# kocvara/Loraine.jl

Hardware: AMD Instinct MI355X
Metric: ms/IP-iteration (Schur assembly + solve), dense SDP n=2000 m=4000 (lower is better)
Workload: dtype f64; 1 GPU; C4 synthetic dense SDP, matrix side 2000, 4000 constraints, kit=0 (assembly + Cholesky + predictor/corrector solves); msz=2000, nvar=4000, seed=20250614, parallelism=1 GPU

## Files before the change

include/loraine_hip.h:

```cpp
#ifndef LORAINE_HIP_H
#define LORAINE_HIP_H

#include <stdint.h>

#ifdef __cplusplus
extern "C" {
#endif

typedef struct lrn_ctx lrn_ctx;

int lrn_create(lrn_ctx** out, int device);
int lrn_destroy(lrn_ctx* ctx);
const char* lrn_last_error(lrn_ctx* ctx);
int lrn_version(void);
int lrn_device_count(void);

int lrn_upload_model(lrn_ctx* ctx, int nlmi, int nvar, const int64_t* msizes,
                     const int64_t* const* AA_colptr, const int64_t* const* AA_rowval,
                     const double* const* AA_nzval,
                     const int64_t* const* B_colptr, const int64_t* const* B_rowval,
                     const double* const* B_nzval,
                     const int64_t* sigmaA, const int64_t* qA,
                     int nlin, const int64_t* Clin_colptr, const int64_t* Clin_rowval,
                     const double* Clin_nzval);
// ... 30 lines not shown
int lrn_matvec(lrn_ctx* ctx, const double* x, double* Ax);
int lrn_matvec_partial(lrn_ctx* ctx, const double* x, double* Ax_partial);
int lrn_prec_setup(lrn_ctx* ctx, int prec, int erank, int aamat, int* info);
int lrn_prec_apply(lrn_ctx* ctx, const double* x, double* Mx);
int lrn_pcg(lrn_ctx* ctx, const double* h, double tol, int maxit, double* x, int* exit_code,
            int* iters);

int lrn_ip_set_c(lrn_ctx* ctx, int ilmi, const double* C);
int lrn_ip_set_iterate(lrn_ctx* ctx, int ilmi, const double* X, const double* S);
int lrn_ip_get_iterate(lrn_ctx* ctx, int ilmi, double* X, double* S);
int lrn_ip_add_diag(lrn_ctx* ctx, int ilmi, int which, double eps);
int lrn_ip_prepare_w(lrn_ctx* ctx, int ilmi, int* info);
int lrn_ip_aa_x(lrn_ctx* ctx, double* out);
int lrn_ip_residual_d(lrn_ctx* ctx, const double* y);
int lrn_ip_rhs_pred(lrn_ctx* ctx, double* out);
int lrn_ip_rhs_pred2(lrn_ctx* ctx, double* aax_out, double* out);
int lrn_ip_rhs_corr(lrn_ctx* ctx, double sigma_mu, double* out);
int lrn_ip_find_step(lrn_ctx* ctx, int predict, double sigma_mu, double tau, const double* dely,
                     double* alpha, double* beta);
int lrn_ip_update(lrn_ctx* ctx, int predict, const double* alpha, const double* beta, double* trXnSn);
int lrn_ip_stats(lrn_ctx* ctx, double* out5);
int lrn_dbg_eigmin(lrn_ctx* ctx, int n, const double* M, double* lam, int* steps);
int lrn_dbg_lanczos(lrn_ctx* ctx, int n, int k, const double* M, double* lam_top, double* U_top,
                    double* lam_min, double* trace, int* steps);

int lrn_dbg_get_block(lrn_ctx* ctx, int il, const char* name, double* out, int* flag);
int lrn_dbg_tridiag_eig(int m, const double* a, const double* b, int k, const double* upper, double width, double* eig,
                        int64_t* evals);

typedef int (*lrn_host_allreduce_fn)(void* user, double* buf, int64_t count, int op);
typedef int (*lrn_host_allgather_fn)(void* user, const double* send, double* recv, int64_t count_per_rank);
int lrn_comm_unique_id(void* id128);
int lrn_comm_init(lrn_ctx* ctx, const void* id128, int rank, int world);
int lrn_comm_init_host(lrn_ctx* ctx, int rank, int world, lrn_host_allreduce_fn allreduce,
                       lrn_host_allgather_fn allgather, void* user);
int lrn_comm_destroy(lrn_ctx* ctx);
int lrn_comm_allreduce(lrn_ctx* ctx, double* buf, int64_t count, int op);

int lrn_get_timing(lrn_ctx* ctx, const char* key, double* ms);
int64_t lrn_get_count(lrn_ctx* ctx, const char* key);
int lrn_mfma_f64_peak(lrn_ctx* ctx, double* tflops);
int lrn_xcc_probe(lrn_ctx* ctx, int nx, int nz, int hold_us, int32_t* out);
int lrn_hbm_copy_peak(lrn_ctx* ctx, int64_t bytes, double* gbps);

int lrn_dbg_gemm(lrn_ctx* ctx, int transA, int transB, int M, int N, int K, double alpha,
                 const double* A, int lda, const double* B, int ldb, double beta, double* C,
                 int ldc, int flags, int ksplit);
int lrn_dbg_product(lrn_ctx* ctx, int kind, int n, const double* A, const double* Bm, double alpha, double a, int tri,
                    double* out0, double* out1, double* scalar);
int lrn_dbg_gemm_plan(int transA, int transB, int M, int N, int K, int lda, int ldb, double beta, int ldc, int flags,
                      int ksplit, int* out6);
int lrn_dbg_schur_chol_plan(int msz, int nd, int rank, int world, int64_t pcap_hint, const int* opts6, int64_t* out10, int* kb,
                            int* ke, int* weights, double* shares3);
int lrn_dbg_mfma_probe(lrn_ctx* ctx, const double* A16x4, const double* B4x16, double* D16x16);
int lrn_dbg_potrf(lrn_ctx* ctx, int n, double* A, int* info);
int lrn_dbg_potrs(lrn_ctx* ctx, int n, const double* A, const double* b, double* x, int* info);
int lrn_dbg_trsm(lrn_ctx* ctx, int n, int nrhs, int trans, const double* A, double* B, int* info);
int lrn_dbg_svd_jacobi(lrn_ctx* ctx, int n, const double* A, double* U_sigma, double* V,
                       double* sigma, int* sweeps);

#ifdef __cplusplus
}
#endif
#endif
```

loraine.jl_amd/_capi.py:

```python
import ctypes as C
import os
import shutil
import subprocess
import sys

import numpy as np

_HERE = os.path.dirname(os.path.abspath(__file__))
LIB_PATH = os.path.join(_HERE, "libloraine_hip.so")

c_ctx = C.c_void_p
PD = C.POINTER(C.c_double)
PI64 = C.POINTER(C.c_int64)
PI = C.POINTER(C.c_int)
PPD = C.POINTER(C.c_void_p)

SIGNATURES = {
    "lrn_create": (C.c_int, [C.POINTER(c_ctx), C.c_int]),
    "lrn_destroy": (C.c_int, [c_ctx]),
    "lrn_last_error": (C.c_char_p, [c_ctx]),
    "lrn_version": (C.c_int, []),
    "lrn_device_count": (C.c_int, []),
    "lrn_upload_model": (C.c_int, [c_ctx, C.c_int, C.c_int, C.c_void_p, PPD, PPD, PPD, PPD, PPD, PPD,
                                   C.c_void_p, C.c_void_p, C.c_int, C.c_void_p, C.c_void_p, C.c_void_p]),
# ... 10 lines not shown
    "lrn_set_lin": (C.c_int, [c_ctx, C.c_void_p, C.c_void_p]),
    "lrn_schur_assemble": (C.c_int, [c_ctx, C.c_int, C.c_void_p]),
    "lrn_schur_get": (C.c_int, [c_ctx, C.c_void_p]),
    "lrn_schur_add_diag": (C.c_int, [c_ctx, C.c_double]),
    "lrn_schur_factor": (C.c_int, [c_ctx, PI]),
    "lrn_schur_solve": (C.c_int, [c_ctx, C.c_void_p, C.c_void_p]),
    "lrn_schur_shard_doubles": (C.c_int64, [c_ctx]),
    "lrn_schur_export_shard": (C.c_int, [c_ctx, C.c_void_p]),
    "lrn_schur_import_all": (C.c_int, [c_ctx, C.c_void_p]),
    "lrn_schur_is_partial_sum": (C.c_int, [c_ctx]),
    "lrn_schur_plan": (C.c_int, [c_ctx, C.c_int, PI]),
    "lrn_schur_export_full": (C.c_int, [c_ctx, C.c_void_p]),
    "lrn_schur_import_full": (C.c_int, [c_ctx, C.c_void_p]),
    "lrn_make_rhs": (C.c_int, [c_ctx, C.c_void_p, PPD, C.c_void_p]),
    "lrn_matvec": (C.c_int, [c_ctx, C.c_void_p, C.c_void_p]),
    "lrn_matvec_partial": (C.c_int, [c_ctx, C.c_void_p, C.c_void_p]),
    "lrn_prec_setup": (C.c_int, [c_ctx, C.c_int, C.c_int, C.c_int, PI]),
    "lrn_prec_apply": (C.c_int, [c_ctx, C.c_void_p, C.c_void_p]),
    "lrn_pcg": (C.c_int, [c_ctx, C.c_void_p, C.c_double, C.c_int, C.c_void_p, PI, PI]),
    "lrn_comm_unique_id": (C.c_int, [C.c_void_p]),
    "lrn_comm_init": (C.c_int, [c_ctx, C.c_void_p, C.c_int, C.c_int]),
    "lrn_comm_init_host": (C.c_int, [c_ctx, C.c_int, C.c_int, C.c_void_p, C.c_void_p, C.c_void_p]),
    "lrn_comm_destroy": (C.c_int, [c_ctx]),
    "lrn_comm_allreduce": (C.c_int, [c_ctx, C.c_void_p, C.c_int64, C.c_int]),
    "lrn_ip_set_c": (C.c_int, [c_ctx, C.c_int, C.c_void_p]),
    "lrn_ip_set_iterate": (C.c_int, [c_ctx, C.c_int, C.c_void_p, C.c_void_p]),
    "lrn_ip_get_iterate": (C.c_int, [c_ctx, C.c_int, C.c_void_p, C.c_void_p]),
    "lrn_ip_add_diag": (C.c_int, [c_ctx, C.c_int, C.c_int, C.c_double]),
    "lrn_ip_prepare_w": (C.c_int, [c_ctx, C.c_int, PI]),
    "lrn_ip_aa_x": (C.c_int, [c_ctx, C.c_void_p]),
    "lrn_ip_residual_d": (C.c_int, [c_ctx, C.c_void_p]),
    "lrn_ip_rhs_pred": (C.c_int, [c_ctx, C.c_void_p]),
    "lrn_ip_rhs_pred2": (C.c_int, [c_ctx, C.c_void_p, C.c_void_p]),
    "lrn_ip_rhs_corr": (C.c_int, [c_ctx, C.c_double, C.c_void_p]),
    "lrn_ip_find_step": (C.c_int, [c_ctx, C.c_int, C.c_double, C.c_double, C.c_void_p, C.c_void_p, C.c_void_p]),
    "lrn_ip_update": (C.c_int, [c_ctx, C.c_int, C.c_void_p, C.c_void_p, C.c_void_p]),
    "lrn_ip_stats": (C.c_int, [c_ctx, C.c_void_p]),
    "lrn_dbg_get_block": (C.c_int, [c_ctx, C.c_int, C.c_char_p, C.c_void_p, PI]),
    "lrn_dbg_tridiag_eig": (C.c_int, [C.c_int, C.c_void_p, C.c_void_p, C.c_int, C.c_void_p, C.c_double, PD, PI64]),
    "lrn_dbg_eigmin": (C.c_int, [c_ctx, C.c_int, C.c_void_p, PD, PI]),
    "lrn_dbg_lanczos": (C.c_int, [c_ctx, C.c_int, C.c_int, C.c_void_p, C.c_void_p, C.c_void_p, PD, PD, PI]),
    "lrn_get_timing": (C.c_int, [c_ctx, C.c_char_p, PD]),
    "lrn_get_count": (C.c_int64, [c_ctx, C.c_char_p]),
    "lrn_mfma_f64_peak": (C.c_int, [c_ctx, PD]),
    "lrn_hbm_copy_peak": (C.c_int, [c_ctx, C.c_int64, PD]),
    "lrn_xcc_probe": (C.c_int, [c_ctx, C.c_int, C.c_int, C.c_int, C.c_void_p]),
    "lrn_dbg_gemm": (C.c_int, [c_ctx, C.c_int, C.c_int, C.c_int, C.c_int, C.c_int, C.c_double, C.c_void_p,
                               C.c_int, C.c_void_p, C.c_int, C.c_double, C.c_void_p, C.c_int, C.c_int, C.c_int]),
    "lrn_dbg_product": (C.c_int, [c_ctx, C.c_int, C.c_int, C.c_void_p, C.c_void_p, C.c_double, C.c_double, C.c_int,
                                  C.c_void_p, C.c_void_p, PD]),
    "lrn_dbg_gemm_plan": (C.c_int, [C.c_int, C.c_int, C.c_int, C.c_int, C.c_int, C.c_int, C.c_int, C.c_double, C.c_int,
                                    C.c_int, C.c_int, PI]),
    "lrn_dbg_schur_chol_plan": (C.c_int, [C.c_int, C.c_int, C.c_int, C.c_int, C.c_int64, PI, PI64, PI, PI, PI, PD]),
    "lrn_dbg_mfma_probe": (C.c_int, [c_ctx, C.c_void_p, C.c_void_p, C.c_void_p]),
    "lrn_dbg_potrf": (C.c_int, [c_ctx, C.c_int, C.c_void_p, PI]),
    "lrn_dbg_potrs": (C.c_int, [c_ctx, C.c_int, C.c_void_p, C.c_void_p, C.c_void_p, PI]),
    "lrn_dbg_trsm": (C.c_int, [c_ctx, C.c_int, C.c_int, C.c_int, C.c_void_p, C.c_void_p, PI]),
    "lrn_dbg_svd_jacobi": (C.c_int, [c_ctx, C.c_int, C.c_void_p, C.c_void_p, C.c_void_p, C.c_void_p, PI]),
}

GEMM_TRI_LOWER, GEMM_TRI_UPPER, GEMM_OFFDIAG_X2, GEMM_SQUARE, GEMM_KSEG_TRI, GEMM_SMALL_TILE = 1, 2, 4, 8, 16, 32
GEMM_KFROM_N, GEMM_KFROM_M, GEMM_KTO_N, GEMM_KTO_M, GEMM_C_MIRROR, GEMM_DYN_MASKS = 64, 128, 1024, 2048, 4096, 131072

_lib = None


class LoraineHipError(RuntimeError):
    pass


def load_library():
    global _lib
    if _lib is not None:
        return _lib
    if not os.path.exists(LIB_PATH) and shutil.which("hipcc") and os.environ.get("LRN_NO_AUTOBUILD") is None:
        csrc = os.path.join(os.path.dirname(os.path.abspath(__file__)), "csrc")
        import fcntl
        with open(os.path.join(csrc, ".build.lock"), "w") as lock:
            fcntl.flock(lock, fcntl.LOCK_EX)
            if not os.path.exists(LIB_PATH):
                print(f"[loraine.jl_amd] {LIB_PATH} missing: running `make -C {csrc}` (hipcc --offload-arch=gfx950)",
                      file=sys.stderr, flush=True)
                subprocess.run(["make", "-C", csrc, "-j8"], check=False, stdout=subprocess.DEVNULL)
    if not os.path.exists(LIB_PATH):
        raise LoraineHipError(
            f"{LIB_PATH} not found: build it with `python -c 'import __graft_entry__ as g; g.build()'` "
            "(hipcc --offload-arch=gfx950). There is no CPU fallback.")
    try:
        import torch
    except ImportError:
        pass
    lib = C.CDLL(LIB_PATH)
    for name, (res, args) in SIGNATURES.items():
        fn = getattr(lib, name)
        fn.restype = res
        fn.argtypes = args
    _lib = lib
    return lib


def ptr(a):
    if a is None:
        return None
    if isinstance(a, int):
        return C.c_void_p(a)
    if isinstance(a, np.ndarray):
        return C.c_void_p(a.ctypes.data)
    if hasattr(a, "data_ptr"):
        if getattr(a, "is_cuda", False):
            import torch
            torch.cuda.current_stream(a.device).synchronize()
        return C.c_void_p(a.data_ptr())
    raise TypeError(type(a))


# ... 10 lines not shown
```

loraine.jl_amd/csrc/api.hip:

```cpp
#include <cstring>

#include "../../include/loraine_hip.h"
#include "ctx.h"
#include "ops.h"
#include "schur_plan.h"

using namespace lrn;

void lrn_free_model(lrn_ctx* c);
namespace lrn {
void prec_free(lrn_ctx* c);
}

extern "C" {

int lrn_version(void) { return 102; }

int lrn_device_count(void) {
  int n = 0;
  if (hipGetDeviceCount(&n) != hipSuccess) {
    (void)hipGetLastError();
    return 0;
  }
  return n;
}

int lrn_create(lrn_ctx** out, int device) {
  if (!out) return LRN_ERR_ARG;
  *out = nullptr;
  int n = lrn_device_count();
  if (n <= 0 || device < 0 || device >= n) return LRN_ERR_HIP;
  if (hipSetDevice(device) != hipSuccess) return LRN_ERR_HIP;
  lrn_ctx* c = new lrn_ctx();
  c->device = device;
  c->profile = false;
  if (hipStreamCreateWithFlags(&c->stream, hipStreamNonBlocking) != hipSuccess ||
      hipEventCreate(&c->ev0) != hipSuccess || hipEventCreate(&c->ev1) != hipSuccess) {
    delete c;
    return LRN_ERR_HIP;
  }
  *out = c;
  return LRN_OK;
}

int lrn_destroy(lrn_ctx* c) {
  if (!c) return LRN_OK;
  (void)hipSetDevice(c->device);
  (void)hipStreamSynchronize(c->stream);
  prec_free(c);
  comm_free(c);
  lrn_free_model(c);
  release(c->info_dev);
  release(c->scratch);
  release(c->jscratch);
  release(c->redbuf);
  release(c->redout);
  release(c->lzbuf);
  release(c->lzbuf2);
  release(c->lxbuf);
  release(c->ezbuf);
  release(c->commvec);
  release(c->commmat);
  release(c->hopbuf);
  release(c->triw);
  release(c->cgpart);
  if (c->pin) (void)hipHostFree(c->pin);
  for (hipEvent_t e : c->pcg_ev) if (e) (void)hipEventDestroy(e);
  (void)hipEventDestroy(c->ev0);
  (void)hipEventDestroy(c->ev1);
  if (c->evA) (void)hipEventDestroy(c->evA);
  if (c->evB) (void)hipEventDestroy(c->evB);
  (void)hipStreamDestroy(c->stream);
  if (c->stream2) (void)hipStreamDestroy(c->stream2);
  if (c->stream3) (void)hipStreamDestroy(c->stream3);
  delete c;
  return LRN_OK;
}

const char* lrn_last_error(lrn_ctx* c) {
  if (!c) return "null context";
  if (const char* g = lrn::gemm_last_error()) {
    if (c->err.find(g) == std::string::npos) c->err += std::string(c->err.empty() ? "" : " | ") + g;
  }
  return c->err.c_str();
}

int lrn_set_option(lrn_ctx* c, const char* key, double value) {
  if (!c || !key) return LRN_ERR_ARG;
  if (!strcmp(key, "dense_threshold")) c->opt.dense_threshold = value;
  else if (!strcmp(key, "profile")) c->profile = value != 0.0;
  else if (!strcmp(key, "t_batch")) { c->opt.t_batch = (long)value; for (auto& b : c->lmi) b.t_cap = b.p_cap = 0; }
  else if (!strcmp(key, "p_batch")) { c->opt.p_batch = (long)value; for (auto& b : c->lmi) b.t_cap = b.p_cap = 0; }
  else if (!strcmp(key, "prec_eig")) c->opt.prec_eig = (int)value;
  else if (!strcmp(key, "pivot_boost")) c->opt.pivot_boost = value;
  else if (!strcmp(key, "schur_chol")) c->opt.schur_chol = (int)value;
  else if (!strcmp(key, "schur_plan")) c->opt.schur_plan = (int)value;
  else if (!strcmp(key, "gemm3_ksplit")) c->opt.gemm3_ksplit = (int)value;
  else if (!strcmp(key, "gemm_no_skip")) c->opt.gemm_no_skip = (int)value;
  else if (!strcmp(key, "gemm_dyn_masks")) c->opt.gemm_dyn_masks = (int)value;
  else if (!strcmp(key, "gemm1_diag")) c->opt.gemm1_diag = (int)value;
  else if (!strcmp(key, "gemm_lab")) c->opt.gemm_lab = (int)value & 127;
  else if (!strcmp(key, "gemm3_sched")) c->opt.gemm3_sched = (int)value;
  else if (!strcmp(key, "gemm3_tile")) c->opt.gemm3_tile = (int)value;
  else if (!strcmp(key, "gemm3_strip")) c->opt.gemm3_strip = (int)value;
  else if (!strcmp(key, "gemm3_stagger")) c->opt.gemm3_stagger = (int)value;
  else if (!strcmp(key, "jacobi_wgs")) c->opt.jacobi_wgs = (int)value;
  else if (!strcmp(key, "jacobi_block")) c->opt.jacobi_block = (int)value;
  else if (!strcmp(key, "jacobi_inner")) c->opt.jacobi_inner = (int)value;
  else if (!strcmp(key, "pair_lanes")) c->opt.pair_lanes = (int)value;
  else if (!strcmp(key, "matvec_sparse")) c->opt.matvec_sparse = (int)value;
  else if (!strcmp(key, "prec_dense")) c->opt.prec_dense = (int)value;
  else if (!strcmp(key, "wmw_pattern_min")) c->opt.wmw_pattern_min = std::max(2, (int)value);
  else if (!strcmp(key, "profile_symv")) c->opt.profile_symv = (int)value;
  else if (!strcmp(key, "profile_ops")) c->opt.profile_ops = (int)value;
  else if (!strcmp(key, "matvec_h")) { c->opt.matvec_h = (int)value; c->hop_version = -1; }
  else if (!strcmp(key, "comm_fail_ensure")) lrn::comm_inject_ensure_failure(c);
  else if (!strcmp(key, "pcg_lookahead")) c->opt.pcg_lookahead = std::max(0, std::min(8, (int)value));
  else if (!strcmp(key, "lowrank_form")) c->opt.lowrank_form = std::max(-1, std::min(1, (int)value));
  else if (!strcmp(key, "cg_lowrank")) {
    c->opt.cg_lowrank = std::max(-1, std::min(1, (int)value));
    c->hop_version = -1;
  }
  else if (!strcmp(key, "cg_factored")) { c->opt.cg_factored = value != 0.0 ? 1 : 0; c->hop_version = -1; }
  else if (!strcmp(key, "hop_max_mb")) { c->opt.hop_max_mb = value < 0.0 ? -1.0 : value; c->hop_version = -1; }
  else if (!strcmp(key, "fac_op_scaled")) { c->opt.fac_op_scaled = std::max(-1, std::min(1, (int)value)); c->hop_version = -1; }
  else if (!strcmp(key, "fac_quadform")) { c->opt.fac_quadform = std::max(-1, std::min(1, (int)value)); c->hop_version = -1; }
  else if (!strcmp(key, "diag_sq_mfma")) c->opt.diag_sq_mfma = std::max(-1, std::min(1, (int)value));
  else if (!strcmp(key, "fac_cross_lds")) c->opt.fac_cross_lds = std::max(-1, std::min(1, (int)value));
  else if (!strcmp(key, "jacobi_cross")) c->opt.jacobi_cross = (int)value;
  else if (!strcmp(key, "jacobi_early")) c->opt.jacobi_early = value;
  else if (!strcmp(key, "eigmin_pair")) c->opt.eigmin_pair = (int)value;
  else if (!strcmp(key, "lz_resident")) c->opt.lz_resident = (int)value;
  else if (!strcmp(key, "lz_res_limit")) {
    if (!(value == value)) return LRN_ERR_ARG;
    c->lz_res_limit = (long long)std::max(1000.0, std::min(2000000.0, value));
  }
  else if (!strcmp(key, "lz_test_withhold")) {
    if (!(value >= 0.0 && value < 1200000.0)) return LRN_ERR_ARG;
    const long code = (long)value;
    const long sel = code / 100000;
    c->lz_wh_left = code % 100000;
    c->lz_wh_run = (int)(sel % 2); c->lz_wh_step = (int)(sel / 2 % 3); c->lz_wh_wg = (int)(sel / 6);
  }
  else if (!strcmp(key, "prepw_streams")) c->opt.prepw_streams = (int)value;
  else if (!strcmp(key, "jacobi_warm")) c->opt.jacobi_warm = value != 0.0;
  else if (!strcmp(key, "nt_mode")) c->opt.nt_mode = (int)value;
  else if (!strcmp(key, "prec_inv")) c->opt.prec_inv = (int)value;
  else if (!strcmp(key, "shard_passes")) c->opt.shard_passes = (int)value;
  else if (!strcmp(key, "shard_products")) c->opt.shard_products = (int)value;
  else if (!strcmp(key, "shard_products_min")) c->opt.shard_products_min = std::max(16, (int)value);
  else if (!strcmp(key, "ns_l0")) c->opt.ns_l0 = value;
  else if (!strcmp(key, "ns_maxit")) c->opt.ns_maxit = (int)value;
  else if (!strcmp(key, "ns_lanczos")) c->opt.ns_lanczos = (int)value;
// ... 406 lines not shown
    std::vector<double> part((size_t)npart);
    rc = copy_out(c, part.data(), dP.p, (size_t)npart * 8);
    double s = 0.0;
    for (int i = 0; i < npart; ++i) s += part[i];
    *scalar = s;
  }
  release(dA); release(dB); release(d0); release(d1); release(dW); release(dP);
  return rc == LRN_OK ? rc : set_error(c, rc, "lrn_dbg_product: kind %d failed", kind);
}

int lrn_dbg_gemm_plan(int transA, int transB, int M, int N, int K, int lda, int ldb, double beta, int ldc, int flags, int ksplit,
                      int* out6) {
  if (!out6) return LRN_ERR_ARG;
  alignas(16) static double dummy[2];
  GemmDesc g;
  g.A = dummy; g.B = dummy; g.C = dummy;
  g.M = M; g.N = N; g.K = K;
  if (!transA) { g.sAm = 1; g.sAk = lda; } else { g.sAm = lda; g.sAk = 1; }
  if (!transB) { g.sBk = 1; g.sBn = ldb; } else { g.sBk = ldb; g.sBn = 1; }
  g.flags = flags;
  if (ksplit > 1 || (flags & GEMM_KSEG_TRI)) {
    g.sCm = 1; g.sCn = M; g.ksplit = ksplit < 1 ? 1 : ksplit; g.sCs = (long)M * N;
    if (flags & GEMM_KSEG_TRI) {
      int ld = 1;
      while ((long)(ld + 1) * (ld + 1) <= K) ++ld;
      g.kseg_ld = ld; g.kseg_cols = ld;
    }
  } else {
    g.sCm = 1; g.sCn = ldc; g.beta = beta;
  }
  GemmPlanInfo info;
  const int rc = gemm_plan_info(g, &info);
  const int v[6] = {info.kernel, info.tile, info.grid_x, info.grid_z, info.dyn_lds, info.slabs};
  for (int i = 0; i < 6; ++i) out6[i] = v[i];
  return rc;
}

int lrn_dbg_schur_chol_plan(int msz, int nd, int rank, int world, int64_t pcap_hint, const int* opts6, int64_t* out10, int* kb,
                            int* ke, int* weights, double* shares3) {
  if (!opts6 || !out10 || !kb || !ke || !weights || !shares3 || msz < 1 || nd < 1 || world < 1 || rank < 0 || rank >= world)
    return LRN_ERR_ARG;
  CholPlanOpts o;
  o.p_batch = opts6[0]; o.gemm3_tile = opts6[1]; o.gemm3_ksplit = opts6[2];
  o.gemm3_sched = opts6[3]; o.gemm3_strip = opts6[4]; o.gemm_no_skip = opts6[5];
  const CholPlan p = plan_chol(msz, nd, rank, world, (long)pcap_hint, o);
  const int64_t v[10] = {p.idle ? -1 : p.c0, p.idle ? -1 : p.c1, p.p_elems, p.ldp, p.P_cap, p.t160 ? 160 : 128,
                         p.ncls,             p.cls[0],           p.cls[1],  p.nslab};
  for (int i = 0; i < 10; ++i) out10[i] = v[i];
  for (int s = 0; s < p.nslab; ++s) { kb[s] = p.kb[s]; ke[s] = p.ke[s]; weights[s] = (int)p.sw.w[s]; }
  shares3[0] = p.gemm1_share; shares3[1] = p.gemm2_share; shares3[2] = p.gemm3_share;
  return LRN_OK;
}

int lrn_dbg_mfma_probe(lrn_ctx* c, const double* A, const double* B, double* D) {
  if (!c || !A || !B || !D) return LRN_ERR_ARG;
  LRN_HIP(c, hipSetDevice(c->device));
  DBuf dA, dB, dD;
  LRN_TRY(ensure(c, dA, 64 * 8));
  LRN_TRY(ensure(c, dB, 64 * 8));
  LRN_TRY(ensure(c, dD, 256 * 8, true));
  LRN_TRY(copy_in(c, dA.p, A, 64 * 8));
  LRN_TRY(copy_in(c, dB.p, B, 64 * 8));
  LRN_TRY(mfma_f64_probe(c->stream, dA.as<double>(), dB.as<double>(), dD.as<double>()));
  int rc = copy_out(c, D, dD.p, 256 * 8);
  release(dA); release(dB); release(dD);
  return rc;
}

static int dbg_factor(lrn_ctx* c, int n, const double* A, DBuf& dA, int* info) {
  DBuf dW;
  LRN_TRY(ensure(c, dA, (size_t)n * n * 8));
  LRN_TRY(ensure(c, dW, chol_work_doubles(n) * 8));
  LRN_TRY(ensure(c, c->info_dev, 64));
  LRN_TRY(copy_in(c, dA.p, A, (size_t)n * n * 8));
  LRN_HIP(c, hipMemsetAsync(c->info_dev.p, 0, 4, c->stream));
  tic(c);
  LRN_TRY(potrf_lower(c->stream, dA.as<double>(), n, n, dW.as<double>(), c->info_dev.as<int>()));
  toc(c, "dbg_potrf");
  int h = 0;
  LRN_TRY(copy_out(c, &h, c->info_dev.p, 4));
  if (info) *info = h;
  release(dW);
  return LRN_OK;
}

int lrn_dbg_potrf(lrn_ctx* c, int n, double* A, int* info) {
  if (!c || !A || n <= 0) return LRN_ERR_ARG;
  LRN_HIP(c, hipSetDevice(c->device));
  DBuf dA;
  LRN_TRY(dbg_factor(c, n, A, dA, info));
  int rc = copy_out(c, A, dA.p, (size_t)n * n * 8);
  release(dA);
  return rc;
}

int lrn_dbg_potrs(lrn_ctx* c, int n, const double* A, const double* b, double* x, int* info) {
  if (!c || !A || !b || !x || n <= 0) return LRN_ERR_ARG;
  LRN_HIP(c, hipSetDevice(c->device));
  DBuf dA, v;
  int inf = 0;
  LRN_TRY(dbg_factor(c, n, A, dA, &inf));
  if (info) *info = inf;
  if (inf != 0) { release(dA); return LRN_OK; }
  LRN_TRY(ensure(c, v, (size_t)(4 * n + 64) * 8, true));
  double* vb = v.as<double>();
  LRN_TRY(copy_in(c, vb, b, (size_t)n * 8));
// ... 25 lines not shown
```

loraine.jl_amd/csrc/ctx.h:

```cpp
#pragma once
#include <map>

#include "chol.h"
#include "lrn_common.h"

namespace lrn { struct Prec; struct Comm; }

struct LmiBlock {
  int msz = 0;
  long nent = 0;
  std::vector<int> sigma;
  std::vector<int> ipos;
  std::vector<long> nnz;
  int qA = 0;
  int nd = 0;
  int q_wave = 0;
  int npos_nz = 0;
  long p_cap = 0, t_cap = 0;
  lrn::DBuf ent_ptr;
  lrn::DBuf ent_r, ent_c;
  lrn::DBuf ent_v;
  lrn::DBuf Adense;
  enum DenseRoute { DENSE_SCALAR = 0, DENSE_STREAM, DENSE_TRI };
  DenseRoute dense_route = DENSE_SCALAR;
// ... 6 lines not shown
  lrn::DBuf cq_j;
  lrn::DBuf cq_v;
  bool sp_ok = false;
  std::vector<int> sp_long_cols;
  lrn::DBuf pc_ptr;
  lrn::DBuf pc_r;
  lrn::DBuf pc_t;
  lrn::DBuf ent_t;
  lrn::DBuf Mv, Zs;
  bool has_B = false;
  long bnnz = 0;
  lrn::DBuf b_ptr, b_col, b_val;
  int lr_khat = 0;
  bool has_V = false;
  long vnnz = 0;
  lrn::DBuf v_ptr, v_col, v_val, v_w;
  bool v_partial = false;
  lrn::DBuf X, S, W, G, Gi, Si, D, DDsi;
  lrn::DBuf Vprev;
  lrn::DBuf Cd, Rd, delX, delS, Xn, Sn, RNT, t0, t1, t2;
  bool resident = false;
  bool have_Vprev = false;
  bool have_W = false, have_G = false;
  lrn::DBuf LXf, LXt, LSf, Yh, Zh, Ki, Bs, TX, Qm, lyap, Bd;
  double ns_c = 1.0;
  bool nt_free = false;
  bool chol_valid = false;
  bool have_Bd = false;
  lrn::DBuf Vd;
  bool have_Vd = false;
  bool factored = false;
  bool hybrid() const { return factored && npos_nz > 0; }
  lrn::DBuf Ys;
  long Ys_version = -1;
  int dg_n = 0;
  lrn::DBuf dg_h, dg_nat, dg_of_pos;
  lrn::DBuf dg_a;
};

struct lrn_ctx;
namespace lrn { void update_shard_bs(lrn_ctx* c); }

struct LrnOptions {
  double dense_threshold = -1.0;
  long t_batch = 0, p_batch = 0;
  int prec_eig = 0;
  double pivot_boost = 1e-12;
  int schur_chol = -1;
  int schur_plan = -1;
  int gemm3_ksplit = 0;
  int gemm_dyn_masks = 0;
  int gemm_lab = 0;
  int gemm1_diag = 1;
  int gemm_no_skip = 0;
  int gemm3_sched = 1;
  int gemm3_strip = 1;
  int gemm3_tile = 0;
  int gemm3_stagger = 0;
  int jacobi_inner = 0;
  int jacobi_wgs = 0;
  int jacobi_block = 0;
  int jacobi_cross = 1;
  int prepw_streams = 1;
  int lz_resident = 1;
  int eigmin_pair = 2;
  double jacobi_early = 3e-8;
  bool jacobi_warm = true;
  int shard_passes = 1;
  int prec_inv = -1;
  int nt_mode = 1;
  double ns_l0 = 2e-3;
  int ns_lanczos = 1;
  int ns_lanczos_min = 1500;
  int ns_dual = -1;
  int ns_maxit = 40;
  double lyap_tol = 1e-12;
  int lyap_maxit = 300;
  int lyap_form = 1;
  int pair_lanes = 0;
  int matvec_sparse = 0;
  int shard_products = 1;
  int shard_products_min = 4096;
  int prec_dense = 0;
  int wmw_pattern_min = 1500;
  int profile_ops = 0;
  int profile_symv = 0;
  int matvec_h = 0;
  int pcg_lookahead = 2;
  int fac_cross_lds = -1;
  int lowrank_form = -1;
  int cg_lowrank = 0;
  int cg_factored = 0;
  double hop_max_mb = -1.0;
  int fac_op_scaled = -1;
  int fac_quadform = -1;
  int diag_sq_mfma = -1;
};

struct lrn_ctx {
  int device = 0;
  LrnOptions opt;
  hipStream_t stream = nullptr;
  hipStream_t stream2 = nullptr;
  std::string err;
  int nlmi = 0, nvar = 0, nlin = 0;
  std::vector<LmiBlock> lmi;
// ... 109 lines not shown
```

loraine.jl_amd/csrc/gemm_f64.hip:

```cpp
#include "lrn_common.h"

#include <algorithm>
#include <cstdlib>
#include <map>
#include <mutex>
#include <tuple>
#include <type_traits>
#include <utility>
#include <vector>

namespace lrn {

static constexpr int BK = 16;
static constexpr int MAX_KSPLIT = 64;

struct GemmParams {
  GemmDesc d;
  int tilesM, tilesN;
  int kchunk;
  int kcols[MAX_KSPLIT + 1];
  int kcols2[MAX_KSPLIT + 1];
  const int2* tile_list;
  const int2* tile_list2;
  int n1, n2;
  int m_org = 0, n_org = 0;
};

#define MFMA_F64_ROW(lane, r) (((lane) >> 4) + 4 * (r))
#define LRN_MFMA_INPLACE(c, a, b) asm volatile("v_mfma_f64_16x16x4_f64 %0, %1, %2, %0" : "+v"(c) : "v"(a), "v"(b))
#define LRN_MFMA_DRAIN() asm volatile("s_nop 15\n\ts_nop 15\n\ts_nop 15" ::: "memory")

template <int BM, bool KC>
__device__ __forceinline__ int lds_idx(int m, int k) {
  return KC ? (m * (BK + 2) + k) : (k * (BM + 16) + m);
}

template <int BM, int BN, bool AKC, bool BKC, bool KSEG, bool EPI>
__global__ __launch_bounds__(256, 2) void gemm_f64_kernel(GemmParams p) {
  constexpr int TM = BM / 32, TN = BN / 32;
  constexpr int EA = BM * BK / 256, EB = BN * BK / 256;
  constexpr int LA = BK * (BM + 16), LB = BK * (BN + 16);
  __shared__ double lds[2 * (LA + LB)];

  const GemmDesc& d = p.d;
  int tm, tn;
  {
    int bid = blockIdx.x, nwg = gridDim.x;
    int q = nwg >> 3, r = nwg & 7, xcd = bid & 7;
    int swz = (xcd < r ? xcd * (q + 1) : r * (q + 1) + (xcd - r) * q) + (bid >> 3);
    int2 tt = p.tile_list[swz];
    tm = tt.x;
    tn = tt.y;
  }
  if (tm < 0) return;
  const int ks = blockIdx.z % d.ksplit;
  const int bz = blockIdx.z / d.ksplit;
  const double* __restrict__ Ag = d.A + (long)bz * d.bA;
  const double* __restrict__ Bg = d.B + (long)bz * d.bB;
  double* __restrict__ Cg = d.C + (long)bz * d.bC + (long)ks * d.sCs;

  const int t = threadIdx.x, lane = t & 63, w = t >> 6;
  const int wm = w & 1, wn = w >> 1;
  const int m0 = tm * BM, n0 = tn * BN;

  long kcur, kend;
  int segc = 0, segcend = 0, segr = 0;
  if (KSEG) {
    segc = p.kcols[ks];
    segcend = p.kcols[ks + 1];
    segr = (segc / 128) * 128;
    kcur = 0; kend = 0;
  } else {
    kcur = (long)ks * p.kchunk;
    kend = kcur + p.kchunk;
    if (kend > d.K) kend = d.K;
    if (d.flags & GEMM_KFROM_N) kcur = n0;
    if (d.flags & GEMM_KFROM_M) kcur = m0;
    if ((d.flags & GEMM_KTO_N) && kend > n0 + BN) kend = n0 + BN;
    if ((d.flags & GEMM_KTO_M) && kend > m0 + BM) kend = m0 + BM;
  }

// ... 311 lines not shown
    const double* sb = sa + LA;
    if (mask != 0u) {
      double fa[BK / 4][TM], fb[BK / 4][TN];
#pragma unroll
      for (int kk = 0; kk < BK / 4; ++kk) {
#pragma unroll
        for (int i = 0; i < TM; ++i) fa[kk][i] = sa[(kk * 4 + fk) * LROW + (2 * i + wm) * 16 + fr];
#pragma unroll
        for (int j = 0; j < TN; ++j) fb[kk][j] = sb[(kk * 4 + fk) * LROW + (2 * j + wn) * 16 + fr];
      }
#pragma unroll
      for (int kk = 0; kk < BK / 4; ++kk)
#pragma unroll
        for (int i = 0; i < TM; ++i)
#pragma unroll
          for (int j = 0; j < TN; ++j)
            if (mask & (1u << (i * 4 + j))) LRN_MFMA_INPLACE(acc[i][j], fa[kk][i], fb[kk][j]);
    }
    __syncthreads();
  };
  auto static_step = [&](auto mc, int kt) __attribute__((always_inline)) {
    constexpr unsigned MK = decltype(mc)::value;
    const int cur = kt & 1;
    if (kt + 1 < nk) issue(kt + 1, cur ^ 1);
    const double* sa = lds + cur * (2 * LA);
    const double* sb = sa + LA;
    asm volatile("; static K-step, block pattern %0" ::"n"(MK) : "memory");
    if (MK != 0u) {
      double fa[2][TM], fb[2][TN];
      auto frags = [&](int kk) __attribute__((always_inline)) {
#pragma unroll
        for (int i = 0; i < TM; ++i)
          if (MK & (0xfu << (4 * i))) fa[kk & 1][i] = sa[(kk * 4 + fk) * LROW + (2 * i + wm) * 16 + fr];
#pragma unroll
        for (int j = 0; j < TN; ++j)
          if (MK & (0x1111u << j)) fb[kk & 1][j] = sb[(kk * 4 + fk) * LROW + (2 * j + wn) * 16 + fr];
      };
      frags(0);
#pragma unroll
      for (int kk = 0; kk < BK / 4; ++kk) {
        if (kk + 1 < BK / 4) frags(kk + 1);
#pragma unroll
        for (int i = 0; i < TM; ++i)
#pragma unroll
          for (int j = 0; j < TN; ++j)
            if (MK & (1u << (i * 4 + j))) LRN_MFMA_INPLACE(acc[i][j], fa[kk & 1][i], fb[kk & 1][j]);
      }
    }
    __syncthreads();
  };
  if (!(d.flags & GEMM_LAB_NO_LOAD)) issue(kt0, kt0 & 1);
  __syncthreads();
  int kt = (d.flags & GEMM_LAB_NO_KLOOP) ? nk : kt0;
  if constexpr (DYN) {
    int head_end = kt0, tail_begin = nk;
    if (smask != 0xffffu) {
      head_end = nk;
    } else {
      if (from_n | from_m) head_end = kt0 + 8 < nk ? kt0 + 8 : nk;
      if (to_n) tail_begin = n0 / BK;
      if (to_m && m0 / BK < tail_begin) tail_begin = m0 / BK;
      if (d.flags & GEMM_NO_SKIP) { head_end = kt0; tail_begin = nk; }
      if (tail_begin < head_end) tail_begin = head_end;
      if (tail_begin > nk) tail_begin = nk;
    }
    for (; kt < head_end; ++kt) masked_step(kt, step_mask(kt));
    for (; kt < tail_begin; ++kt) fast_step(kt);
    for (; kt < nk; ++kt) masked_step(kt, step_mask(kt));
  } else {
    int e[12];
#pragma unroll
    for (int q = 0; q < 12; ++q) e[q] = kt0;
    if (smask == 0xffffu) {
      if ((from_n | from_m) && !(d.flags & GEMM_NO_SKIP)) {
        const int w0 = kt0 + (from_n ? wn : wm);
        e[0] = w0;
        if (from_n) { e[1] = w0 + 2; e[2] = w0 + 4; e[3] = w0 + 6; }
        else { e[4] = w0 + 2; e[5] = w0 + 4; e[6] = w0 + 6; }
      }
    } else if (!(d.flags & GEMM_NO_SKIP)) {
      if ((smask & ~0x1111u) == 0u) e[1] = nk;
      else if ((smask & ~0x000fu) == 0u) e[4] = nk;
      else if ((smask & ~0x08ceu) == 0u) e[7] = nk;
      else if ((smask & ~0x7310u) == 0u) e[9] = nk;
      else if ((smask & ~0x3333u) == 0u) e[2] = nk;
      else if ((smask & ~0x00ffu) == 0u) e[5] = nk;
      else if ((smask & ~0x8cefu) == 0u) e[8] = nk;
      else if ((smask & ~0xf731u) == 0u) e[10] = nk;
      else if ((smask & ~0x7777u) == 0u) e[3] = nk;
      else if ((smask & ~0x0fffu) == 0u) e[6] = nk;
    }
#define LRN_PATTERN_LOOP(q, m)                                                             \
    {                                                                                      \
      const int end = e[q] < nk ? e[q] : nk;                                               \
      for (; kt < end; ++kt) static_step(std::integral_constant<unsigned, m>{}, kt);       \
    }
    LRN_PATTERN_LOOP(0, 0x0000u)
    LRN_PATTERN_LOOP(1, 0x1111u) LRN_PATTERN_LOOP(2, 0x3333u) LRN_PATTERN_LOOP(3, 0x7777u)
    LRN_PATTERN_LOOP(4, 0x000fu) LRN_PATTERN_LOOP(5, 0x00ffu) LRN_PATTERN_LOOP(6, 0x0fffu)
    LRN_PATTERN_LOOP(7, 0x08ceu) LRN_PATTERN_LOOP(8, 0x8cefu)
    LRN_PATTERN_LOOP(9, 0x7310u) LRN_PATTERN_LOOP(10, 0xf731u)
#undef LRN_PATTERN_LOOP
    for (; kt < nk; ++kt) fast_step(kt);
  }
  LRN_MFMA_DRAIN();
  if (d.flags & GEMM_LAB_NO_STORE) return;
// ... 900 lines not shown
```

loraine.jl_amd/csrc/lrn_common.h:

```cpp
#pragma once
#include <hip/hip_runtime.h>

#include <cstdint>
#include <cstdio>
#include <cstring>
#include <string>
#include <vector>

#define LRN_OK 0
#define LRN_ERR_ARG (-1)
#define LRN_ERR_HIP (-2)
#define LRN_ERR_STATE (-3)
#define LRN_ERR_NOMEM (-4)

typedef double v4f64 __attribute__((ext_vector_type(4)));

namespace lrn {

__host__ __device__ inline int shard_owner(int blk, int world) {
  int r = blk % world;
  return ((blk / world) & 1) ? world - 1 - r : r;
}
__host__ __device__ inline int shard_global_block(int rank, int lb, int world) {
  return lb * world + ((lb & 1) ? world - 1 - rank : rank);
}

static inline unsigned nb(long n, long cap = 4096) {
  long b = (n + 255) / 256;
  return (unsigned)(b < 1 ? 1 : (b > cap ? cap : b));
}

struct DBuf {
  void* p = nullptr;
  size_t bytes = 0;
  size_t* acct = nullptr;
  template <class T> T* as() const { return reinterpret_cast<T*>(p); }
};

enum : int {
  GEMM_TRI_LOWER = 1,
  GEMM_TRI_UPPER = 2,
  GEMM_OFFDIAG_X2 = 4,
  GEMM_SQUARE = 8,
  GEMM_KSEG_TRI = 16,
  GEMM_SMALL_TILE = 32,
  GEMM_KFROM_N = 64,
  GEMM_KFROM_M = 128,
  GEMM_C_PACKED = 256,
  GEMM_KTO_N = 1024,
  GEMM_KTO_M = 2048,
  GEMM_C_MIRROR = 4096,
  GEMM_DIAG_LOWER = 8192,
  GEMM_DIAG_UPPER = 16384,
  GEMM_TILE160 = 65536,
  GEMM_DYN_MASKS = 131072,
  GEMM_NO_SKIP = 32768,
  GEMM_DIAG_LOWER_Z = 262144,
  GEMM_LAB_SAME_CHUNK = 1 << 25,
  GEMM_LAB_NO_STORE = 1 << 20,
  GEMM_LAB_NO_KLOOP = 1 << 21,
  GEMM_LAB_NO_LOAD = 1 << 22,
  GEMM_LAB_ONE_WG = 1 << 23,
  GEMM_SQUARE_BLOCKSUM = 1 << 26,
  GEMM_KFLAT = 512,
};

__host__ __device__ inline int packed_S(int m) { return (m + 15) & ~15; }
__host__ __device__ inline long packed_diag_elems(int m) { return 16L * m; }
__host__ __device__ inline long packed_off_base(int c, int S) {
  const long q = c >> 4;
  return 16L * (q * S - 8L * q * (q + 1)) + (long)(c - 16 * q) * (S - 16 * (q + 1));
}
__host__ __device__ inline long packed_total_elems(int m) { return packed_diag_elems(m) + packed_off_base(m, packed_S(m)); }
__host__ __device__ inline long packed_lower_offset(int r, int c, int S, long Kd) {
  const int q = c >> 4;
  if ((r >> 4) == q) return 16L * c + (r - 16 * q);
  return Kd + packed_off_base(c, S) + (r - 16 * (q + 1));
}

struct GemmDesc {
  const double* A = nullptr;
  const double* B = nullptr;
  double* C = nullptr;
  double* C2 = nullptr;
  int M = 0, N = 0, K = 0;
  long sAm = 0, sAk = 0, sBk = 0, sBn = 0, sCm = 0, sCn = 0;
  long bA = 0, bB = 0, bC = 0;
  int batch = 1;
  double alpha = 1.0, beta = 0.0;
  int flags = 0;
  int ksplit = 1;
  long sCs = 0;
  int kseg_ld = 0, kseg_cols = 0;
  int pk_m = 0;
  long pk_cstride = 16;
  int pk_off = 0;
  long kflat_cstride = 16;
  const int* kflat_kb = nullptr;
  const int* kflat_ke = nullptr;
  long kflat_total = 0, kflat_diag = 0;
  int kflat_nsd = 0;
  int tile_class = 0;
  unsigned long long* lab_trace = nullptr;
  int kstagger = 0;
  const double* blk_w = nullptr;
  int blk_k = 0;
};

int gemm(hipStream_t st, const GemmDesc& d);
struct SlabSrc {
// ... 20 lines not shown
```

loraine.jl_amd/csrc/schur_dense.hip:

```cpp
#include "ops.h"
#include "schur_plan.h"

namespace lrn {

static constexpr int TS = 128;
static constexpr int BK_CHUNK = 16;

__global__ __launch_bounds__(256) void dense_sparse_gather_kernel(
    const long* __restrict__ ptr, const int* __restrict__ er, const int* __restrict__ ec,
    const double* __restrict__ ev, const double* __restrict__ T, int msz, int s0, int ns, int p_lo,
    int p_end, const int* __restrict__ hidx, double* __restrict__ H, int ldh) {
  const int s = blockIdx.y;
  if (s >= ns) return;
  const int pj = p_lo + blockIdx.x * 256 + threadIdx.x;
  if (pj >= p_end) return;
  const double* Ts = T + (long)s * msz * msz;
  double acc = 0.0;
  for (long f = ptr[pj]; f < ptr[pj + 1]; ++f) {
    int p = er[f], q = ec[f];
    int tp = p / TS, tq = q / TS;
    double t;
    if (tp == tq) t = Ts[(long)p + (long)q * msz];
    else if (tp > tq) t = 0.5 * Ts[(long)p + (long)q * msz];
    else t = 0.5 * Ts[(long)q + (long)p * msz];
// ... 94 lines not shown
  if (need > avail) return false;
  if (c->opt.p_batch <= 0 && c->world == 1) {
    const long big = std::min<long>(tri_p_batch(b.msz, true), b.nd);
    if (big > pcap && need + (double)(big - pcap) * mm * 8.0 + 0.10 * (double)total_b <= avail / 0.92) *pcap_out = big;
  }
  return true;
}

__global__ void tril_inplace_kernel(double* __restrict__ L, int m) {
  long total = (long)m * m;
  for (long e = (long)blockIdx.x * blockDim.x + threadIdx.x; e < total; e += (long)gridDim.x * blockDim.x) {
    int i = (int)(e % m), j = (int)(e / m);
    if (i < j) L[e] = 0.0;
  }
}

static int factor_w(lrn_ctx* c, LmiBlock& b, bool* ok) {
  const int m = b.msz;
  const long mm = (long)m * m;
  *ok = false;
  LRN_TRY(ensure(c, c->wchol, (2 * (size_t)mm + chol_work_doubles(m)) * 8));
  double* Lw = c->wchol.as<double>();
  double* Ut = Lw + mm;
  double* cw = Ut + mm;
  tic(c);
  LRN_HIP(c, hipMemcpyAsync(Lw, b.W.p, (size_t)mm * 8, hipMemcpyDeviceToDevice, c->stream));
  LRN_HIP(c, hipMemsetAsync(c->info_dev.p, 0, 8, c->stream));
  LRN_TRY(potrf_lower(c->stream, Lw, m, m, cw, c->info_dev.as<int>()));
  int h_info = 0;
  LRN_HIP(c, hipMemcpyAsync(&h_info, c->info_dev.p, 4, hipMemcpyDeviceToHost, c->stream));
  LRN_HIP(c, hipStreamSynchronize(c->stream));
  if (h_info != 0) {
    c->counts["wchol_fail"] += 1;
    return LRN_OK;
  }
  hipLaunchKernelGGL(transpose_lower_kernel, dim3((m + 31) / 32, (m + 31) / 32), dim3(256), 0, c->stream, Lw, m, Ut);
  hipLaunchKernelGGL(tril_inplace_kernel, dim3(nb(mm)), dim3(256), 0, c->stream, Lw, m);
  toc(c, "wchol");
  *ok = true;
  return LRN_OK;
}

static int chol_lab12(const LrnOptions& o) {
  return (o.gemm_no_skip ? GEMM_NO_SKIP : 0) | (o.gemm_dyn_masks ? GEMM_DYN_MASKS : 0) | ((o.gemm_lab & 15) << 20);
}
static GemmDesc chol_gemm1(const lrn_ctx* c, const CholPlan& pl, int m, const double* Ad, const double* Ut, double* P, int a,
                           int nbat) {
  const long mm = (long)m * m, off = (long)pl.c0 + (long)pl.c0 * m;
  GemmDesc g1;
  g1.A = Ad + (long)a * mm + off; g1.sAm = 1; g1.sAk = m; g1.bA = mm;
  g1.B = Ut + off; g1.sBk = m; g1.sBn = 1; g1.bB = 0;
  g1.C = P; g1.sCm = pl.ldp; g1.sCn = 1; g1.bC = pl.p_elems;
  g1.M = g1.K = m - pl.c0; g1.N = pl.c1 - pl.c0; g1.batch = nbat;
  g1.flags = GEMM_TRI_LOWER | GEMM_KFROM_N | chol_lab12(c->opt) | (c->opt.gemm1_diag ? GEMM_DIAG_LOWER_Z : 0);
  if (c->opt.gemm_lab & 32) g1.bA = 0;
  if (c->opt.gemm_lab & 16) g1.flags &= ~GEMM_KFROM_N;
  return g1;
}
static GemmDesc chol_gemm2(const lrn_ctx* c, const CholPlan& pl, int m, const double* Ut, const double* P, double* T,
                           long cstride, int a, int nbat) {
  const long off = (long)pl.c0 + (long)pl.c0 * m;
  GemmDesc g2;
  g2.A = Ut + off; g2.sAm = 1; g2.sAk = m; g2.bA = 0;
  g2.B = P; g2.sBk = pl.ldp; g2.sBn = 1; g2.bB = pl.p_elems;
  g2.C = T + (long)a * 16; g2.sCm = 1; g2.sCn = m; g2.bC = 16;
  g2.pk_cstride = cstride;
  g2.M = g2.K = m - pl.c0; g2.N = pl.c1 - pl.c0; g2.batch = nbat;
  g2.flags = GEMM_TRI_LOWER | GEMM_KFROM_M | GEMM_C_PACKED | chol_lab12(c->opt);
  if (c->opt.gemm_lab & 32) g2.bB = 0;
  if (c->opt.gemm_lab & 16) g2.flags &= ~GEMM_KFROM_M;
  g2.pk_m = m;
  g2.pk_off = pl.c0;
  return g2;
}
static GemmDesc chol_gemm3(const lrn_ctx* c, const CholPlan& pl, int m, int nd, const double* T, long cstride, double* slabs) {
  GemmDesc g3;
  g3.A = T; g3.sAm = 16; g3.sAk = 1;
  g3.B = T; g3.sBk = 1; g3.sBn = 16;
  g3.kflat_cstride = cstride;
  g3.C = slabs; g3.sCm = 1; g3.sCn = nd;
  g3.M = nd; g3.N = nd;
  g3.flags = GEMM_TRI_LOWER | GEMM_KFLAT | GEMM_DIAG_LOWER | (c->opt.gemm_no_skip ? GEMM_NO_SKIP : 0) |
             (pl.t160 ? GEMM_TILE160 : 0) | ((c->opt.gemm_lab & 64) ? GEMM_LAB_SAME_CHUNK : 0);
  g3.kflat_total = packed_total_elems(m); g3.kflat_diag = packed_diag_elems(m); g3.kflat_nsd = 1;
  g3.kflat_kb = pl.kb; g3.kflat_ke = pl.ke;
  g3.kstagger = c->opt.gemm3_stagger;
  g3.ksplit = pl.nslab; g3.sCs = (long)nd * nd;
  return g3;
}

static int assemble_dense_chol(lrn_ctx* c, LmiBlock& b, long pcap_hint) {
  const int m = b.msz, nd = b.nd;
  CholPlanOpts po;
  po.p_batch = c->opt.p_batch; po.gemm3_tile = c->opt.gemm3_tile; po.gemm3_ksplit = c->opt.gemm3_ksplit;
  po.gemm3_sched = c->opt.gemm3_sched; po.gemm3_strip = c->opt.gemm3_strip; po.gemm_no_skip = c->opt.gemm_no_skip;
  const CholPlan pl = plan_chol(m, nd, c->rank, c->world, pcap_hint, po);
  c->timing["gemm1_share"] = pl.gemm1_share;
  c->timing["gemm2_share"] = pl.gemm2_share;
  c->timing["gemm3_share"] = pl.gemm3_share;
  const long cstride = 16L * nd;
  LRN_TRY(ensure(c, c->P, (size_t)pl.P_cap * std::max<long>(pl.p_elems, 1) * 8));
  LRN_TRY(claim_T(c, b, 1, (size_t)(packed_total_elems(m) / 16) * cstride * 8));
  if (pl.nslab > 0) LRN_TRY(ensure(c, c->slabs, (size_t)pl.nslab * nd * nd * 8));
  HdTarget hd;
  LRN_TRY(hd_target(c, b, &hd));
  const double* Ut = c->wchol.as<double>() + (long)m * m;
  double* P = c->P.as<double>();
  double* T = c->T.as<double>();
  for (int a = 0; a < nd && !pl.idle; a += (int)pl.P_cap) {
    const int nbat = std::min((int)pl.P_cap, nd - a);
    tic(c);
    LRN_TRY(gemm(c->stream, chol_gemm1(c, pl, m, b.Adense.as<double>(), Ut, P, a, nbat)));
    toc(c, "gemm1");
    tic(c);
    LRN_TRY(gemm(c->stream, chol_gemm2(c, pl, m, Ut, P, T, cstride, a, nbat)));
    toc(c, "gemm2");
  }
  GemmDesc g3 = chol_gemm3(c, pl, m, nd, T, cstride, c->slabs.as<double>());
  for (int l = 0; l < pl.ncls; ++l) {
    tic(c);
    g3.tile_class = pl.cls[l];
// ... 154 lines not shown
```

Measured before the change: 976.2 ms.

## Deal diagonal-tile lower-triangle blocks evenly across four waves in MFMA GEMM

For triangular diagonal tiles in the batched Cholesky-based Schur GEMMs, the kernel now gives each of the four waves exactly nine 16x16 MFMA blocks of the 36 lower-triangle blocks, instead of the interleaved ownership that leaves waves with unequal work. This removes load imbalance on diagonal tiles, where the slowest wave sets the tile time. The cost is a separate compile-time-specialised k-loop path with more accumulators and register pressure, plus explicit zero stores for the masked upper blocks. A debug API exposes the owner map for checking.

```diff
diff --git a/include/loraine_hip.h b/include/loraine_hip.h
--- a/include/loraine_hip.h
+++ b/include/loraine_hip.h
@@ -106,6 +106,7 @@
                       int ksplit, int* out6);
 int lrn_dbg_schur_chol_plan(int msz, int nd, int rank, int world, int64_t pcap_hint, const int* opts6, int64_t* out10, int* kb,
                             int* ke, int* weights, double* shares3);
+int lrn_dbg_tile_deal(int kind, int even, int* owner64);
 int lrn_dbg_mfma_probe(lrn_ctx* ctx, const double* A16x4, const double* B4x16, double* D16x16);
 int lrn_dbg_potrf(lrn_ctx* ctx, int n, double* A, int* info);
 int lrn_dbg_potrs(lrn_ctx* ctx, int n, const double* A, const double* b, double* x, int* info);
diff --git a/loraine.jl_amd/_capi.py b/loraine.jl_amd/_capi.py
--- a/loraine.jl_amd/_capi.py
+++ b/loraine.jl_amd/_capi.py
@@ -86,6 +86,7 @@
     "lrn_dbg_gemm_plan": (C.c_int, [C.c_int, C.c_int, C.c_int, C.c_int, C.c_int, C.c_int, C.c_int, C.c_double, C.c_int,
                                     C.c_int, C.c_int, PI]),
     "lrn_dbg_schur_chol_plan": (C.c_int, [C.c_int, C.c_int, C.c_int, C.c_int, C.c_int64, PI, PI64, PI, PI, PI, PD]),
+    "lrn_dbg_tile_deal": (C.c_int, [C.c_int, C.c_int, PI]),
     "lrn_dbg_mfma_probe": (C.c_int, [c_ctx, C.c_void_p, C.c_void_p, C.c_void_p]),
     "lrn_dbg_potrf": (C.c_int, [c_ctx, C.c_int, C.c_void_p, PI]),
     "lrn_dbg_potrs": (C.c_int, [c_ctx, C.c_int, C.c_void_p, C.c_void_p, C.c_void_p, PI]),
@@ -95,6 +96,7 @@
 
 GEMM_TRI_LOWER, GEMM_TRI_UPPER, GEMM_OFFDIAG_X2, GEMM_SQUARE, GEMM_KSEG_TRI, GEMM_SMALL_TILE = 1, 2, 4, 8, 16, 32
 GEMM_KFROM_N, GEMM_KFROM_M, GEMM_KTO_N, GEMM_KTO_M, GEMM_C_MIRROR, GEMM_DYN_MASKS = 64, 128, 1024, 2048, 4096, 131072
+GEMM_EVEN_DEAL = 524288
 
 _lib = None
 
diff --git a/loraine.jl_amd/csrc/api.hip b/loraine.jl_amd/csrc/api.hip
--- a/loraine.jl_amd/csrc/api.hip
+++ b/loraine.jl_amd/csrc/api.hip
@@ -3,6 +3,7 @@
 #include "../../include/loraine_hip.h"
 #include "ctx.h"
 #include "ops.h"
+#include "partial_tiles.h"
 #include "schur_plan.h"
 
 using namespace lrn;
@@ -99,6 +100,7 @@
   else if (!strcmp(key, "gemm_no_skip")) c->opt.gemm_no_skip = (int)value;
   else if (!strcmp(key, "gemm_dyn_masks")) c->opt.gemm_dyn_masks = (int)value;
   else if (!strcmp(key, "gemm1_diag")) c->opt.gemm1_diag = (int)value;
+  else if (!strcmp(key, "gemm_even_deal")) c->opt.gemm_even_deal = (int)value;
   else if (!strcmp(key, "gemm_lab")) c->opt.gemm_lab = (int)value & 127;
   else if (!strcmp(key, "gemm3_sched")) c->opt.gemm3_sched = (int)value;
   else if (!strcmp(key, "gemm3_tile")) c->opt.gemm3_tile = (int)value;
@@ -611,6 +613,11 @@
   return LRN_OK;
 }
 
+int lrn_dbg_tile_deal(int kind, int even, int* owner64) {
+  if (!owner64) return LRN_ERR_ARG;
+  return tile_deal_owners(kind, even != 0, owner64) ? LRN_OK : LRN_ERR_ARG;
+}
+
 int lrn_dbg_mfma_probe(lrn_ctx* c, const double* A, const double* B, double* D) {
   if (!c || !A || !B || !D) return LRN_ERR_ARG;
   LRN_HIP(c, hipSetDevice(c->device));
diff --git a/loraine.jl_amd/csrc/ctx.h b/loraine.jl_amd/csrc/ctx.h
--- a/loraine.jl_amd/csrc/ctx.h
+++ b/loraine.jl_amd/csrc/ctx.h
@@ -82,6 +82,7 @@
   int gemm_dyn_masks = 0;
   int gemm_lab = 0;
   int gemm1_diag = 1;
+  int gemm_even_deal = 1;
   int gemm_no_skip = 0;
   int gemm3_sched = 1;
   int gemm3_strip = 1;
diff --git a/loraine.jl_amd/csrc/gemm_f64.hip b/loraine.jl_amd/csrc/gemm_f64.hip
--- a/loraine.jl_amd/csrc/gemm_f64.hip
+++ b/loraine.jl_amd/csrc/gemm_f64.hip
@@ -1,4 +1,5 @@
 #include "lrn_common.h"
+#include "partial_tiles.h"
 
 #include <algorithm>
 #include <cstdlib>
@@ -27,6 +28,14 @@
 };
 
 #define MFMA_F64_ROW(lane, r) (((lane) >> 4) + 4 * (r))
+template <class F, int... I>
+__device__ __forceinline__ void static_for_impl(F&& f, std::integer_sequence<int, I...>) {
+  (f(std::integral_constant<int, I>{}), ...);
+}
+template <int N, class F>
+__device__ __forceinline__ void static_for(F&& f) {
+  static_for_impl(f, std::make_integer_sequence<int, N>{});
+}
 #define LRN_MFMA_INPLACE(c, a, b) asm volatile("v_mfma_f64_16x16x4_f64 %0, %1, %2, %0" : "+v"(c) : "v"(a), "v"(b))
 #define LRN_MFMA_DRAIN() asm volatile("s_nop 15\n\ts_nop 15\n\ts_nop 15" ::: "memory")
 
@@ -444,6 +453,88 @@
   if (!(d.flags & GEMM_LAB_NO_LOAD)) issue(kt0, kt0 & 1);
   __syncthreads();
   int kt = (d.flags & GEMM_LAB_NO_KLOOP) ? nk : kt0;
+  if constexpr (!DYN) {
+    const bool whole = m0 + BM <= d.M && n0 + BN <= d.N;
+    const bool diag_tile = tm == tn && m0 == n0 && whole &&
+                           (EPI ? (d.flags & GEMM_C_PACKED) && !(d.flags & GEMM_SQUARE) : (d.flags & GEMM_DIAG_LOWER_Z) != 0);
+    if (diag_tile && (d.flags & GEMM_EVEN_DEAL) &&
+        !(d.flags & (GEMM_NO_SKIP | GEMM_LAB_NO_STORE | GEMM_LAB_NO_KLOOP | GEMM_LAB_NO_LOAD))) {
+      auto store_plain = [&](int m, int n, double v) __attribute__((always_inline)) {
+        double* cp = Cg + (long)m * d.sCm + (long)n * d.sCn;
+        if (d.beta != 0.0) v += d.beta * (*cp);
+        *cp = v;
+      };
+      auto dealt = [&](auto wc) __attribute__((always_inline)) {
+        constexpr int W = decltype(wc)::value;
+        constexpr int NB = DIAG_DEAL_BLOCKS;
+        constexpr bool MIR = EPI;
+        v4f64 c[NB];
+#pragma unroll
+        for (int q = 0; q < NB; ++q) c[q] = (v4f64){0.0, 0.0, 0.0, 0.0};
+        for (; kt < nk; ++kt) {
+          const int cur = kt & 1;
+          if (kt + 1 < nk) issue(kt + 1, cur ^ 1);
+          const double* sa = lds + cur * (2 * LA);
+          const double* sb = sa + LA;
+#pragma unroll
+          for (int kk = 0; kk < BK / 4; ++kk) {
+            double fa[8], fb[8];
+            static_for<8>([&](auto bc) __attribute__((always_inline)) {
+              constexpr int b = decltype(bc)::value;
+              if constexpr (diag_deal_uses_bm(W, b, MIR)) fa[b] = sa[(kk * 4 + fk) * LROW + b * 16 + fr];
+              if constexpr (diag_deal_uses_bn(W, b, MIR)) fb[b] = sb[(kk * 4 + fk) * LROW + b * 16 + fr];
+            });
+            static_for<NB>([&](auto qc) __attribute__((always_inline)) {
+              constexpr int q = decltype(qc)::value;
+              constexpr TileBlock b = diag_deal_block(W, q, MIR);
+              c[q] = __builtin_amdgcn_mfma_f64_16x16x4f64(fa[b.bm], fb[b.bn], c[q], 0, 0, 0);
+            });
+          }
+          __syncthreads();
+        }
+        if constexpr (EPI) {
+          const long pkS = packed_S(d.pk_m), S16 = pkS >> 4, kd16 = packed_diag_elems(d.pk_m > 0 ? d.pk_m : 1) >> 4;
+          const int qb = (m0 + d.pk_off) >> 4, rbb = (n0 + d.pk_off) >> 4;
+          static_for<NB>([&](auto qc) __attribute__((always_inline)) {
+            constexpr int q = decltype(qc)::value;
+            constexpr TileBlock b = diag_deal_block(W, q, MIR);
+            const long qq = qb + b.bm, rb = rbb + b.bn;
+            const long below = kd16 + qq * pkS - 8 * qq * (qq + 1) - qq - 1, percol = S16 - qq - 1;
+#pragma unroll
+            for (int r = 0; r < 4; ++r) {
+              const int cc = MFMA_F64_ROW(lane, r);
+              const long chunk = rb == qq ? 16 * qq + cc : below + cc * percol + rb;
+              Cg[chunk * d.pk_cstride + fr] = d.alpha * c[q][r];
+            }
+          });
+        } else {
+          static_for<NB>([&](auto qc) __attribute__((always_inline)) {
+            constexpr int q = decltype(qc)::value;
+            constexpr TileBlock b = diag_deal_block(W, q, MIR);
+#pragma unroll
+            for (int r = 0; r < 4; ++r)
+              store_plain(m0 + b.bm * 16 + MFMA_F64_ROW(lane, r), n0 + b.bn * 16 + fr, d.alpha * c[q][r]);
+          });
+        }
+      };
+      if (w == 0) dealt(std::integral_constant<int, 0>{});
+      else if (w == 1) dealt(std::integral_constant<int, 1>{});
+      else if (w == 2) dealt(std::integral_constant<int, 2>{});
+      else dealt(std::integral_constant<int, 3>{});
+      if constexpr (!EPI) {
+#pragma unroll
+        for (int i = 0; i < TM; ++i)
+#pragma unroll
+          for (int j = 0; j < TN; ++j) {
+            if (!(zmask & (1u << (i * 4 + j)))) continue;
+#pragma unroll
+            for (int r = 0; r < 4; ++r)
+              store_plain(m0 + (2 * i + wm) * 16 + MFMA_F64_ROW(lane, r), n0 + (2 * j + wn) * 16 + fr, d.alpha * 0.0);
+          }
+      }
+      return;
+    }
+  }
   if constexpr (DYN) {
     int head_end = kt0, tail_begin = nk;
     if (smask != 0xffffu) {
diff --git a/loraine.jl_amd/csrc/lrn_common.h b/loraine.jl_amd/csrc/lrn_common.h
--- a/loraine.jl_amd/csrc/lrn_common.h
+++ b/loraine.jl_amd/csrc/lrn_common.h
@@ -56,6 +56,7 @@
   GEMM_DYN_MASKS = 131072,
   GEMM_NO_SKIP = 32768,
   GEMM_DIAG_LOWER_Z = 262144,
+  GEMM_EVEN_DEAL = 524288,
   GEMM_LAB_SAME_CHUNK = 1 << 25,
   GEMM_LAB_NO_STORE = 1 << 20,
   GEMM_LAB_NO_KLOOP = 1 << 21,
diff --git a/loraine.jl_amd/csrc/partial_tiles.h b/loraine.jl_amd/csrc/partial_tiles.h
--- /dev/null
+++ b/loraine.jl_amd/csrc/partial_tiles.h
@@ -0,0 +1,56 @@
+#pragma once
+#include <hip/hip_runtime.h>
+
+namespace lrn {
+
+struct TileBlock {
+  int bm, bn;
+};
+
+static constexpr int DIAG_DEAL_BLOCKS = 9;
+
+__host__ __device__ constexpr TileBlock diag_deal_block(int w, int q, bool mirror) {
+  int r = 0, c = 0;
+  if (w < 3) {
+    r = (w == 1 ? 2 : 5) + q / 3;
+    c = (w == 2 ? 3 : 0) + q % 3;
+  } else {
+    const int base = 3 * (q / 3), e = q % 3;
+    r = base + (e > 0 ? 1 : 0);
+    c = base + (e == 2 ? 1 : 0);
+  }
+  return mirror ? TileBlock{c, r} : TileBlock{r, c};
+}
+__host__ __device__ constexpr bool diag_deal_uses_bm(int w, int bm, bool mirror) {
+  for (int q = 0; q < DIAG_DEAL_BLOCKS; ++q)
+    if (diag_deal_block(w, q, mirror).bm == bm) return true;
+  return false;
+}
+__host__ __device__ constexpr bool diag_deal_uses_bn(int w, int bn, bool mirror) {
+  for (int q = 0; q < DIAG_DEAL_BLOCKS; ++q)
+    if (diag_deal_block(w, q, mirror).bn == bn) return true;
+  return false;
+}
+
+__host__ __device__ constexpr int interleaved_owner(int bm, int bn) { return (bm & 1) | ((bn & 1) << 1); }
+
+inline bool tile_deal_owners(int kind, bool even, int* owner) {
+  if (kind != 0 && kind != 1) return false;
+  const bool mirror = kind == 1;
+  for (int e = 0; e < 64; ++e) owner[e] = -1;
+  if (even) {
+    for (int w = 0; w < 4; ++w)
+      for (int q = 0; q < DIAG_DEAL_BLOCKS; ++q) {
+        const TileBlock b = diag_deal_block(w, q, mirror);
+        if (owner[b.bm * 8 + b.bn] != -1) return false;
+        owner[b.bm * 8 + b.bn] = w;
+      }
+  } else {
+    for (int bm = 0; bm < 8; ++bm)
+      for (int bn = 0; bn < 8; ++bn)
+        if (mirror ? bn >= bm : bm >= bn) owner[bm * 8 + bn] = interleaved_owner(bm, bn);
+  }
+  return true;
+}
+
+}
diff --git a/loraine.jl_amd/csrc/schur_dense.hip b/loraine.jl_amd/csrc/schur_dense.hip
--- a/loraine.jl_amd/csrc/schur_dense.hip
+++ b/loraine.jl_amd/csrc/schur_dense.hip
@@ -170,7 +170,8 @@
   g1.B = Ut + off; g1.sBk = m; g1.sBn = 1; g1.bB = 0;
   g1.C = P; g1.sCm = pl.ldp; g1.sCn = 1; g1.bC = pl.p_elems;
   g1.M = g1.K = m - pl.c0; g1.N = pl.c1 - pl.c0; g1.batch = nbat;
-  g1.flags = GEMM_TRI_LOWER | GEMM_KFROM_N | chol_lab12(c->opt) | (c->opt.gemm1_diag ? GEMM_DIAG_LOWER_Z : 0);
+  g1.flags = GEMM_TRI_LOWER | GEMM_KFROM_N | chol_lab12(c->opt) | (c->opt.gemm1_diag ? GEMM_DIAG_LOWER_Z : 0) |
+             (c->opt.gemm_even_deal ? GEMM_EVEN_DEAL : 0);
   if (c->opt.gemm_lab & 32) g1.bA = 0;
   if (c->opt.gemm_lab & 16) g1.flags &= ~GEMM_KFROM_N;
   return g1;
@@ -184,7 +185,7 @@
   g2.C = T + (long)a * 16; g2.sCm = 1; g2.sCn = m; g2.bC = 16;
   g2.pk_cstride = cstride;
   g2.M = g2.K = m - pl.c0; g2.N = pl.c1 - pl.c0; g2.batch = nbat;
-  g2.flags = GEMM_TRI_LOWER | GEMM_KFROM_M | GEMM_C_PACKED | chol_lab12(c->opt);
+  g2.flags = GEMM_TRI_LOWER | GEMM_KFROM_M | GEMM_C_PACKED | chol_lab12(c->opt) | (c->opt.gemm_even_deal ? GEMM_EVEN_DEAL : 0);
   if (c->opt.gemm_lab & 32) g2.bB = 0;
   if (c->opt.gemm_lab & 16) g2.flags &= ~GEMM_KFROM_M;
   g2.pk_m = m;
```

New measurement: 975.2 ms (median of 2 runs). No clear change (-0.1%).
